# zju3dv/Diffuman4D

Measured on NVIDIA H100. Metric: unet_window_denoise_steps_per_sec, higher is better.
Workload: dtype bf16

## Files before the change

### diffuman4d_b200/_lib.py

```python
from __future__ import annotations

import ctypes as C
import os

_HERE = os.path.dirname(os.path.abspath(__file__))
LIB_PATH = os.path.join(_HERE, "libd4d.so")

EXPORTS = [
    "d4d_last_error", "d4d_version", "d4d_create", "d4d_destroy", "d4d_load_weight", "d4d_finalize_weights",
    "d4d_num_weights", "d4d_weight_key", "d4d_unet_forward", "d4d_profile_forward", "d4d_workspace_bytes", "d4d_forward_launches",
    "d4d_denoise_window", "d4d_denoise_window_dpm", "d4d_assemble_input", "d4d_cfg_ddim_step", "d4d_cfg_dpm_step",
    "d4d_op_gemm", "d4d_op_gemm_kv_scatter", "d4d_op_conv3x3",
    "d4d_op_attention", "d4d_op_groupnorm", "d4d_op_conv3x3_groupnorm", "d4d_op_conv_resample", "d4d_op_layernorm", "d4d_op_pose_conv0", "d4d_op_pose_conv", "d4d_debug_tap", "d4d_exchange_alloc",
    "d4d_exchange_open", "d4d_unet_forward_sharded", "d4d_denoise_window_sharded", "d4d_denoise_window_dpm_sharded",
    "d4d_window_exchange", "d4d_op_window_scatter", "d4d_denoise_window_unipc", "d4d_cfg_unipc_step",
    "d4d_op_conv_tiled", "d4d_conv_tile_choice", "d4d_op_gemm_tiled", "d4d_gemm_tile_choice",
    "d4d_denoise_window_pndm", "d4d_cfg_pndm_step", "d4d_denoise_window_deis", "d4d_cfg_deis_step",
    "d4d_denoise_window_dpm_single", "d4d_cfg_dpm_single_step",
    "d4d_denoise_window_cfg_split", "d4d_denoise_window_dpm_cfg_split", "d4d_denoise_window_unipc_cfg_split",
    "d4d_denoise_window_pndm_cfg_split", "d4d_denoise_window_deis_cfg_split", "d4d_denoise_window_dpm_single_cfg_split",
    "d4d_denoise_window_cfg_grid", "d4d_denoise_window_dpm_cfg_grid", "d4d_denoise_window_unipc_cfg_grid",
    "d4d_denoise_window_pndm_cfg_grid", "d4d_denoise_window_deis_cfg_grid", "d4d_denoise_window_dpm_single_cfg_grid",
]


class D4DConfig(C.Structure):
    _fields_ = [
        ("in_channels", C.c_int32), ("out_channels", C.c_int32), ("block_out_channels", C.c_int32 * 4),
        ("layers_per_block", C.c_int32), ("num_heads", C.c_int32 * 4), ("has_attn2", C.c_int32 * 4),
        ("use_linear_projection", C.c_int32), ("norm_num_groups", C.c_int32), ("norm_eps", C.c_float),
        ("flip_sin_to_cos", C.c_int32), ("freq_shift", C.c_float), ("num_3d_attn_blocks", C.c_int32),
# ... 99 lines not shown
    l.d4d_assemble_input.argtypes = [vp, vp, vp, vp, vp, vp, vp, i32, i32, i32, i32, i32, vp, vp, vp]
    l.d4d_cfg_ddim_step.argtypes = [vp, vp, vp, vp, vp, C.POINTER(D4DSched), f32, i32, i32, i32, i32, vp, vp]
    l.d4d_cfg_dpm_step.argtypes = [vp, vp, vp, vp, vp, vp, vp, vp, C.POINTER(D4DDpmSched), f32, i32, i32, i32, i32, vp, vp]
    l.d4d_cfg_unipc_step.argtypes = [vp, vp, vp, vp, vp, vp, vp, vp, vp, vp, C.POINTER(D4DUniPCSched), f32, i32, i32, i32,
                                     i32, vp, vp]
    l.d4d_cfg_pndm_step.argtypes = [vp, vp, vp, vp, vp, vp, vp, vp, vp, vp, vp, vp, C.POINTER(D4DPndmSched), f32, i32,
                                    i32, i32, i32, vp, vp]
    l.d4d_cfg_deis_step.argtypes = [vp, vp, vp, vp, vp, vp, vp, vp, vp, C.POINTER(D4DDeisSched), f32, i32, i32, i32, i32,
                                    vp, vp]
    l.d4d_cfg_dpm_single_step.argtypes = [vp, vp, vp, vp, vp, vp, vp, vp, vp, vp, C.POINTER(D4DDpmSingleSched), f32, i32,
                                          i32, i32, i32, vp, vp]
    l.d4d_op_gemm.argtypes = [vp, i32, i32, vp, i32, i32, vp, i32, i32, f32p, vp, i32, i32, vp, i32, vp, i32, i32,
                              i32, f32, i32, vp, i32, vp]
    l.d4d_op_gemm_tiled.argtypes = [vp, i32, i32, vp, i32, i32, vp, i32, i32, f32p, vp, i32, i32, vp, i32, vp, i32, i32,
                                    i32, f32, i32, i32, vp, i32, vp]
    l.d4d_gemm_tile_choice.argtypes = [i32, i32, i32, i32, i32, i32, C.POINTER(C.c_int), C.POINTER(C.c_int)]
    l.d4d_op_gemm_kv_scatter.argtypes = [vp, i32, i32, vp, i32, i32, vp, i32, i32, i32, C.c_int64, C.c_int64, C.c_int64,
                                         i32, vp, i32, vp]
    l.d4d_op_conv3x3.argtypes = [vp, i32, i32, i32, i32, vp, i32, f32p, vp, i32, vp, i32, vp, i32, vp, vp]
    l.d4d_op_conv_tiled.argtypes = [vp, i32, i32, i32, i32, vp, i32, f32p, vp, i32, vp, i32, vp, i32, i32, i32, vp, vp]
    l.d4d_conv_tile_choice.argtypes = [i32, i32, i32, i32, i32, i32, i32, C.POINTER(C.c_int), C.POINTER(C.c_int)]
    l.d4d_op_attention.argtypes = [vp, vp, vp, i32, vp, i32, i32, i32, i32, i32, f32, i32, i32, vp]
    l.d4d_op_groupnorm.argtypes = [vp, i32, vp, i32, i32, i32, i32, f32, f32p, f32p, i32, vp, vp, vp]
    l.d4d_op_conv3x3_groupnorm.argtypes = [vp, i32, i32, i32, i32, vp, i32, f32p, vp, i32, f32, f32p, f32p, i32, vp, vp, vp,
                                           vp]
    l.d4d_op_conv_resample.argtypes = [vp, i32, i32, i32, i32, vp, i32, f32p, i32, i32, i32, vp, vp, vp]
    l.d4d_op_layernorm.argtypes = [vp, i32, i32, f32, f32p, f32p, vp, vp]
    l.d4d_op_pose_conv0.argtypes = [vp, i32, i32, i32, vp, f32p, vp, vp]
    l.d4d_op_pose_conv.argtypes = [vp, i32, i32, i32, i32, vp, f32p, i32, i32, i32, vp, vp]
    l.d4d_debug_tap.argtypes = [vp, vp, vp, vp, C.POINTER(C.c_int32), i32, i32, i32, i32, i32, i32, vp, C.c_char_p,
                                C.POINTER(C.c_int32), vp]
# ... 30 lines not shown
```

### diffuman4d_b200/csrc/d4d_api.cu

```cuda
#include <new>
#include <stdexcept>

#include "unet.h"

namespace d4d {
static thread_local std::string g_last_error;
void set_error(const std::string& msg) { g_last_error = msg; }
}

struct d4d_handle {
  d4d::Model* model;
};

using d4d::bf16;

#define D4D_API_BEGIN try {
#define D4D_API_END                                        \
  }                                                        \
  catch (const std::bad_alloc&) {                          \
    d4d::set_error("out of host memory");                  \
    return 2;                                              \
  }                                                        \
  catch (const std::exception& e) {                        \
    d4d::set_error(std::string("internal error: ") + e.what()); \
// ... 105 lines not shown
  d4d::StepArgs a;
  const int hw = height * width;
  a.noise = static_cast<const bf16*>(noise); a.latents = static_cast<const bf16*>(latents);
  a.mask = static_cast<const bf16*>(cond_mask);
  a.timestep_indices = reinterpret_cast<const long long*>(timestep_indices);
  a.F = F; a.chw = 4 * hw; a.hw = hw; a.cfg = cfg; a.guidance = guidance_scale;
  a.out = static_cast<bf16*>(latents_out);
  a.ts_out = reinterpret_cast<long long*>(timestep_indices_out);
  return a;
}
}

extern "C" {

const char* d4d_last_error(void) { return d4d::g_last_error.c_str(); }
int d4d_version(void) { return 114; }

int d4d_create(const d4d_config* cfg, int device, d4d_handle** out) {
  D4D_API_BEGIN
  D4D_REQUIRE(cfg != nullptr && out != nullptr, "null argument");
  *out = nullptr;
  D4D_REQUIRE(cfg->layers_per_block >= 1 && cfg->layers_per_block <= 4, "layers_per_block");
  D4D_REQUIRE(cfg->out_channels >= 1 && cfg->out_channels <= 16, "out_channels must be in [1,16]");
  D4D_REQUIRE(cfg->in_channels >= 1 && cfg->in_channels <= 16, "in_channels must be in [1,16]");
  D4D_REQUIRE(cfg->norm_num_groups >= 1 && cfg->norm_num_groups <= 64, "norm_num_groups");
  for (int i = 0; i < 4; ++i) {
    const int c = cfg->block_out_channels[i], hds = cfg->num_heads[i];
    D4D_REQUIRE(c > 0 && c % 64 == 0, "block_out_channels must be positive multiples of 64");
    D4D_REQUIRE(c % cfg->norm_num_groups == 0, "channels must be divisible by norm_num_groups");
    D4D_REQUIRE(hds > 0 && c % hds == 0, "channels must be divisible by the number of heads");
    D4D_REQUIRE(c / hds <= 192 && (c / hds) % 8 == 0, "head_dim must be a multiple of 8 and <= 192");
// ... 247 lines not shown
  D4D_API_END
}

int d4d_op_gemm(const void* A, int lda, int K1, const void* A2, int lda2, int K2, const void* W, int M, int N,
                const float* bias, const void* rowvec, int ld_rowvec, int rows_per_image, const void* residual,
                int ld_res, void* out, int ldo, int geglu, int act, float out_scale, int block_n, int64_t* stats,
                int stats_rows, void* stream) {
  return d4d_op_gemm_tiled(A, lda, K1, A2, lda2, K2, W, M, N, bias, rowvec, ld_rowvec, rows_per_image, residual, ld_res, out,
                           ldo, geglu, act, out_scale, block_n, 0, stats, stats_rows, stream);
}

int d4d_op_gemm_tiled(const void* A, int lda, int K1, const void* A2, int lda2, int K2, const void* W, int M, int N,
                      const float* bias, const void* rowvec, int ld_rowvec, int rows_per_image, const void* residual,
                      int ld_res, void* out, int ldo, int geglu, int act, float out_scale, int block_n, int schedule,
                      int64_t* stats, int stats_rows, void* stream) {
  D4D_API_BEGIN
  d4d::GemmDesc d;
  d.A = static_cast<const bf16*>(A); d.lda = lda; d.K1 = K1;
  d.A2 = static_cast<const bf16*>(A2); d.lda2 = lda2; d.K2 = K2;
  d.Wt = static_cast<const bf16*>(W); d.M = M; d.N = N; d.bias = bias;
  d.rowvec = static_cast<const bf16*>(rowvec); d.ld_rowvec = ld_rowvec; d.rows_per_image = rows_per_image;
  d.residual = static_cast<const bf16*>(residual); d.ld_res = ld_res;
  d.out = static_cast<bf16*>(out); d.ldo = ldo; d.geglu = geglu; d.act = act; d.out_scale = out_scale; d.block_n = block_n;
  d.schedule = schedule;
  d.stats = reinterpret_cast<long long*>(stats); d.stats_rows = stats_rows;
  D4D_REQUIRE(M > 0, "empty GEMM");
  d4d::GemmLaunch L;
  if (int rc = d4d::gemm_prepare(d, &L)) return rc;
  return d4d::gemm_run(L, static_cast<cudaStream_t>(stream));
  D4D_API_END
}

int d4d_gemm_tile_choice(int M, int N, int K1, int K2, int geglu, int sms, int* block_n, int* schedule) {
  D4D_API_BEGIN
  D4D_REQUIRE(M > 0 && N > 0 && K1 > 0 && K2 >= 0 && sms > 0 && block_n && schedule, "gemm_tile_choice arguments");
  d4d::GemmDesc d;
  D4D_REQUIRE(K2 == 0 || K1 % 64 == 0, "two-source GEMM needs K1 % 64 == 0");
  d.M = M; d.N = N; d.K1 = K1 + K2; d.geglu = geglu;
  int block_m = 0;
  return d4d::gemm_choose_tile(d, sms, &block_m, block_n, schedule);
  D4D_API_END
}

int d4d_op_gemm_kv_scatter(const void* A, int lda, int K, const void* W, int M, int N, void* out, int ldo, int kv_col0,
                           int kv_ld, int64_t rows_local, int64_t rows_global, int64_t row_offset, int world,
                           void* const* kv_dst, int block_n, void* stream) {
  D4D_API_BEGIN
  D4D_REQUIRE(M > 0, "empty GEMM");
  D4D_REQUIRE(world >= 1 && world <= 8, "K/V scatter: world must be in [1, 8]");
  D4D_REQUIRE(kv_dst != nullptr, "K/V scatter: null destination buffer");
  d4d::GemmDesc d;
  d.A = static_cast<const bf16*>(A); d.lda = lda; d.K1 = K; d.Wt = static_cast<const bf16*>(W); d.M = M; d.N = N;
  d.out = static_cast<bf16*>(out); d.ldo = ldo; d.block_n = block_n;
  d.kv_world = world; d.kv_col0 = kv_col0; d.kv_ld = kv_ld;
  d.kv_rows_local = rows_local; d.kv_rows_global = rows_global; d.kv_row_offset = row_offset;
// ... 348 lines not shown
```

### diffuman4d_b200/csrc/gemm_wgmma.cu

```cuda
#include "kernels.h"
#include "wgmma.cuh"

namespace d4d {

namespace {

constexpr int BLOCK_M = 128;
constexpr int BLOCK_K = 64;
constexpr int A_BYTES = BLOCK_M * BLOCK_K * 2;
constexpr int BAR_BYTES = 1024;
constexpr int NUM_THREADS = 384;
constexpr int MAX_SMEM = 227 * 1024;

constexpr int SLAB_COLS = 32;
constexpr int SLAB_BYTES = 64 * SLAB_COLS * 2;

template <int BN, int MI, bool kStaged, bool kPingPong>
struct GemmCfg {
  static constexpr int TILE_A_BYTES = kPingPong ? A_BYTES : MI * A_BYTES;
  static constexpr int STAGE_BYTES = TILE_A_BYTES + BN * BLOCK_K * 2;
  static constexpr int STAGING_BYTES = kStaged ? 2 * 64 * MI * BN * 2 : 0;
  static constexpr int STAGES_FIT = (MAX_SMEM - 1024 - BAR_BYTES - STAGING_BYTES) / STAGE_BYTES;
  static constexpr int STAGES = STAGES_FIT > 8 ? 8 : STAGES_FIT;
  static constexpr int SMEM = 1024 + BAR_BYTES + STAGES * STAGE_BYTES + STAGING_BYTES;
};

struct TileCoord {
  int m0;
  int n_img0, y0, x0;
  int pa, pb;
};

template <bool kConv>
__device__ __forceinline__ void tile_coords(const GemmKernelArgs& a, int m_tile, TileCoord& t) {
  if (!kConv) {
    t.m0 = m_tile * BLOCK_M;
    t.n_img0 = t.y0 = t.x0 = 0;
    t.pa = t.pb = 0;
  } else {
    const int ph = a.n_phases > 1 ? m_tile / a.tiles_per_phase : 0;
    m_tile -= ph * a.tiles_per_phase;
    t.pa = ph >> 1;
    t.pb = ph & 1;
    int tx = m_tile % a.tiles_x;
    int r = m_tile / a.tiles_x;
    int ty = r % a.tiles_y;
    int tn = r / a.tiles_y;
    t.m0 = 0;
    t.x0 = tx * a.BW;
    t.y0 = ty * a.BH;
    t.n_img0 = tn * a.BN;
  }
}

template <bool kConv>
__device__ __forceinline__ void row_of(const GemmKernelArgs& a, const TileCoord& tc, int rr, long long& row, int& img,
// ... 13 lines not shown
    img = n;
  }
}

enum : int { E_BIAS = 1, E_ROWVEC = 2, E_ACT = 4, E_RES = 8, E_STATS = 16, E_KV = 32, E_ALL = 63, E_STAGED_ALL = E_ALL & ~E_KV };
__host__ __device__ constexpr bool gemm_staged(bool conv, int epi) { return !conv && !(epi & E_KV); }

constexpr int ORDER_BAR = 3;

template <int BN, int MI, bool kGeglu, bool kConv, int kEpi, bool kPingPong>
__global__ void __launch_bounds__(NUM_THREADS, 1)
gemm_wgmma_kernel(const __grid_constant__ CUtensorMap tmap_a, const __grid_constant__ CUtensorMap tmap_a2,
                  const __grid_constant__ CUtensorMap tmap_b, const __grid_constant__ CUtensorMap tmap_c,
                  const __grid_constant__ CUtensorMap tmap_r, const GemmKernelArgs a) {
  constexpr bool kStaged = gemm_staged(kConv, kEpi);
  static_assert(MI == 1 || (kConv && MI == 2) || kPingPong, "256-row tiles: conv mode only (a plain tile is 128 rows)");
  static_assert(!kPingPong || (kStaged && MI == 2), "ping-pong: staged plain GEMMs, one warpgroup per 128-row tile");
  using Cfg = GemmCfg<BN, MI, kStaged, kPingPong>;
  constexpr int STAGES = Cfg::STAGES;
  extern __shared__ uint8_t smem_raw[];
  uint8_t* smem = reinterpret_cast<uint8_t*>((reinterpret_cast<uintptr_t>(smem_raw) + 1023) & ~uintptr_t(1023));
  uint64_t* full = reinterpret_cast<uint64_t*>(smem);
  uint64_t* empty = full + STAGES;
  uint64_t* res_full = empty + STAGES;
  uint8_t* ring = smem + BAR_BYTES;

  const int warp = __shfl_sync(0xffffffffu, threadIdx.x >> 5, 0);
  const int lane = threadIdx.x & 31;
  const int total_tiles = a.m_tiles * a.n_tiles;

  if (threadIdx.x == 0) {
// ... 45 lines not shown
      }
    }
    return;
  }

  setmaxnreg_inc<232>();
  const int wg = (warp >> 2) - 1;
  const int wq = warp & 3;
  const bool wg_leader = (threadIdx.x & 127) == 0;
  const int wg_row0 = kPingPong ? 0 : wg * 64 * MI;
  const int r_base = wg_row0 + wq * 16 + (lane >> 2);
  const int c_base = 2 * (lane & 3);
  const uint32_t ring_u32 = smem_u32(ring);
  constexpr int STG_BLOCK = 64 * BN * 2;
  const bool staged = kStaged && a.staged;
  uint8_t* stg = ring + STAGES * Cfg::STAGE_BYTES + wg * MI * STG_BLOCK;
  const uint32_t stg_u32 = smem_u32(stg) + (r_base - wg_row0) * 64 + c_base * 2;
  const int stg_xor = (lane >> 3) & 3;
  const bool has_res = (kEpi & E_RES) && !kGeglu && a.residual != nullptr;
  const int out_cols = kGeglu ? a.N / 2 : a.N;
  uint32_t res_phase = 0;

  int stage = 0;
  uint32_t phase = 0;
  const auto skip_stages = [&](int n) {
    stage += n;
    while (stage >= STAGES) { stage -= STAGES; phase ^= 1; }
  };
  if (kPingPong && wg == 1) {
    skip_stages(a.k_blocks);
    named_barrier_arrive(ORDER_BAR, 256);
  }
  const int tile_step = kPingPong ? 2 * gridDim.x : gridDim.x;
  float acc[MI][BN / 2];
  for (int tile = blockIdx.x + (kPingPong ? wg * gridDim.x : 0); tile < total_tiles; tile += tile_step) {
    const int m_tile = tile / a.n_tiles;
    const int n_tile = tile % a.n_tiles;
    TileCoord tc;
    tile_coords<kConv>(a, m_tile, tc);
    const int n0 = n_tile * a.block_n;
    const int ocol0 = kGeglu ? n0 / 2 : n0;
    const int ocols = min(kGeglu ? a.block_n / 2 : a.block_n, out_cols - ocol0);
    const int n_slabs = (ocols + SLAB_COLS - 1) / SLAB_COLS;
    const int orow0 = tc.m0 + wg_row0;
    const int live_blocks = staged ? max(0, min(MI, (a.M - orow0 + 63) / 64)) : 0;

    if (kPingPong) named_barrier_sync(ORDER_BAR + wg, 256);
    int prev_stage = -1;
    for (int kb = 0; kb < a.k_blocks; ++kb) {
      mbar_wait_nocall(&full[stage], phase);
      const uint32_t sa = ring_u32 + stage * Cfg::STAGE_BYTES + wg_row0 * 128;
      const uint32_t sb = ring_u32 + stage * Cfg::STAGE_BYTES + Cfg::TILE_A_BYTES;
      const uint64_t adesc = make_wgmma_desc(sa, 16, 1024);
      const uint64_t bdesc = make_wgmma_desc(sb, 16, 1024);
      wgmma_fence();
#pragma unroll
      for (int k = 0; k < BLOCK_K / 16; ++k) {
        const int scale_d = (kb | k) != 0 ? 1 : 0;
#pragma unroll
        for (int mi = 0; mi < MI; ++mi) {
          const uint64_t ad = adesc + 512 * mi + 2 * k, bd = bdesc + 2 * k;
          if constexpr (BN == 64) wgmma_ss_n64(acc[mi], ad, bd, scale_d);
          else if constexpr (BN == 128) wgmma_ss_n128(acc[mi], ad, bd, scale_d);
          else if constexpr (BN == 160) wgmma_ss_n160(acc[mi], ad, bd, scale_d);
          else if constexpr (BN == 192) wgmma_ss_n192(acc[mi], ad, bd, scale_d);
          else wgmma_ss_n256(acc[mi], ad, bd, scale_d);
        }
      }
      wgmma_commit();
      if (kb == 0 && staged && wg_leader) {
        bulk_wait_group_read<0>();
        if (has_res && live_blocks > 0) {
          mbar_expect_tx(&res_full[wg], live_blocks * n_slabs * SLAB_BYTES);
          for (int mi = 0; mi < live_blocks; ++mi)
            for (int s = 0; s < n_slabs; ++s)
              tma_load_2d(stg + mi * STG_BLOCK + s * SLAB_BYTES, &tmap_r, &res_full[wg], ocol0 + s * SLAB_COLS, orow0 + 64 * mi);
        }
      }
      wgmma_wait<1>();
      if (prev_stage >= 0 && wg_leader) mbar_arrive(&empty[prev_stage]);
      prev_stage = stage;
      if (++stage == STAGES) { stage = 0; phase ^= 1; }
    }
    if (kPingPong) {
      if (tile + gridDim.x < total_tiles) named_barrier_arrive(ORDER_BAR + (wg ^ 1), 256);
      skip_stages(a.k_blocks);
    }
    wgmma_wait<0>();
#pragma unroll
    for (int mi = 0; mi < MI; ++mi) wgmma_fence_regs(acc[mi]);
    if (wg_leader) mbar_arrive(&empty[prev_stage]);

    if (staged) {
      named_barrier_sync(1 + wg, 128);
      if (has_res && live_blocks > 0) {
        mbar_wait_nocall(&res_full[wg], res_phase);
        res_phase ^= 1;
      }
    }
#pragma unroll
    for (int mi = 0; mi < MI; ++mi) {
      auto stg_addr = [&](int j, int h) {
        return stg_u32 + mi * STG_BLOCK + h * 8 * 64 + (j >> 2) * SLAB_BYTES + (((j & 3) ^ stg_xor) << 4);
      };
      float (&accm)[BN / 2] = acc[mi];
      long long rows[2];
      int imgs[2];
      bool valid[2];
      row_of<kConv>(a, tc, r_base + 64 * mi, rows[0], imgs[0], valid[0]);
      row_of<kConv>(a, tc, r_base + 64 * mi + 8, rows[1], imgs[1], valid[1]);
      if constexpr (kGeglu) {
        const bool has_bias = (kEpi & E_BIAS) && a.bias != nullptr;
#pragma unroll
        for (int p = 0; p < BN / 16; ++p) {
          if (16 * p >= a.block_n || n0 + 16 * p >= a.N) break;
          float2 ba = make_float2(0.f, 0.f), bg = make_float2(0.f, 0.f);
          if (has_bias) {
            ba = __ldg(reinterpret_cast<const float2*>(a.bias + n0 + 16 * p + c_base));
// ... 67 lines not shown
              s0 += __shfl_xor_sync(0xffffffffu, s0, m);
              s1 += __shfl_xor_sync(0xffffffffu, s1, m);
              q0 += __shfl_xor_sync(0xffffffffu, q0, m);
              q1 += __shfl_xor_sync(0xffffffffu, q1, m);
            }
            if (stats_on && lane < 4) {
              unsigned long long* st = reinterpret_cast<unsigned long long*>(a.stats) + (static_cast<size_t>(stats_img) * a.N + col) * 2;
              atomicAdd(st + 0, static_cast<unsigned long long>(__float2ll_rn(s0 * kGnSumScale)));
              atomicAdd(st + 1, static_cast<unsigned long long>(__float2ll_rn(q0 * kGnSqScale)));
              atomicAdd(st + 2, static_cast<unsigned long long>(__float2ll_rn(s1 * kGnSumScale)));
              atomicAdd(st + 3, static_cast<unsigned long long>(__float2ll_rn(q1 * kGnSqScale)));
            }
          }
        }
      }
    }
    if (staged) {
      fence_proxy_async_smem();
      named_barrier_sync(1 + wg, 128);
      if (wg_leader && live_blocks > 0) {
        for (int mi = 0; mi < live_blocks; ++mi)
          for (int s = 0; s < n_slabs; ++s)
            tma_store_2d(&tmap_c, stg + mi * STG_BLOCK + s * SLAB_BYTES, ocol0 + s * SLAB_COLS, orow0 + 64 * mi);
        bulk_commit_group();
      }
    }
  }
  if (staged && wg_leader) bulk_wait_group<0>();
}

}

namespace {

void conv_out_grid(const GemmDesc& d, int* oh, int* ow, int* phases) {
  *oh = d.conv_kind == 1 ? d.H / 2 : d.H;
  *ow = d.conv_kind == 1 ? d.W / 2 : d.W;
  *phases = d.conv_kind == 3 ? 4 : 1;
}
// ... 8 lines not shown
  return t;
}

}

constexpr int kOperandWeight = 128;
constexpr int kMinKBlocks256 = 16;
constexpr int kEpilogueWeight = 3072;

namespace {
bool pingpong_width(int bn, bool geglu) { return bn == 128 || (bn == 64 && !geglu); }
}

int gemm_choose_tile(const GemmDesc& d, int sms, int* block_m, int* block_n, int* schedule) {
  D4D_REQUIRE(d.block_m == 0 || d.block_m == 128 || d.block_m == 256, "block_m must be 0 (automatic), 128 or 256");
  D4D_REQUIRE(d.block_m != 256 || d.conv, "256-row tiles: convolutions only (a plain GEMM stages a 128-row tile for its TMA store)");
  D4D_REQUIRE(d.block_m != 256 || d.block_n <= 0 || d.block_n == 128 || d.block_n == 160,
              "256-row tiles run at block_n 128 or 160 (the accumulators of wider tiles do not fit the register file)");
  D4D_REQUIRE(d.schedule == 0 || d.schedule == kSchedCooperative || d.schedule == kSchedPingPong,
              "schedule must be 0 (automatic), 1 (cooperative) or 2 (ping-pong)");
  const bool pp_ok = !d.conv && d.kv_world == 0;
  D4D_REQUIRE(d.schedule != kSchedPingPong || pp_ok, "ping-pong: plain GEMMs without the K/V scatter only");
  D4D_REQUIRE(d.schedule != kSchedPingPong || d.block_n <= 0 || pingpong_width(d.block_n, d.geglu),
              "ping-pong runs at block_n 64 or 128 (GEGLU: 128; wider accumulators do not fit the register file)");
  int oh = 0, ow = 0, phases = 1;
  if (d.conv) conv_out_grid(d, &oh, &ow, &phases);
  D4D_REQUIRE(!d.conv || (d.n_img > 0 && oh > 0 && ow > 0), "empty conv");
  const auto best_tile = [&](bool pingpong, int* bm, int* bn) {
    long long best_cost = -1;
    for (int r : {128, 256}) {
      if (d.block_m > 0 ? r != d.block_m : (r == 256 && !d.conv)) continue;
      if (pingpong && r != 128) continue;
      const int k_blocks = d.conv ? (d.conv_kind >= 2 ? 4 : 9) * ((d.Cin + BLOCK_K - 1) / BLOCK_K) : 0;
      const long long m_tiles = d.conv ? conv_tile(r, d.n_img, oh, ow).tiles * phases : (static_cast<long long>(d.M) + r - 1) / r;
      for (int c : {64, 128, 160, 192, 256}) {
        if (d.block_n > 0) c = d.block_n;
        else if ((d.geglu && c % 64 != 0) || (pingpong && !pingpong_width(c, d.geglu))) continue;
        const long long n_tiles = (d.N + c - 1) / c, tiles = m_tiles * n_tiles;
        const bool fits = r == 128 || ((c == 128 || c == 160) && (d.block_m == 256 || (tiles >= sms && k_blocks >= kMinKBlocks256)));
        if (fits) {
          const long long waves = (tiles + sms - 1) / sms;
          const long long cost = waves * (static_cast<long long>(r) * c + kOperandWeight * (r + c)) + (n_tiles * c - d.N) * (r / 2);
          if (best_cost < 0 || cost <= best_cost) { best_cost = cost; *bm = r; *bn = c; }
        }
        if (d.block_n > 0) break;
      }
    }
    return best_cost >= 0;
  };
  const auto plain_time = [&](bool pingpong, int bn) {
    const long long k_blocks = (d.K1 + BLOCK_K - 1) / BLOCK_K + (d.A2 ? (d.K2 + BLOCK_K - 1) / BLOCK_K : 0);
    const long long tiles = ((static_cast<long long>(d.M) + BLOCK_M - 1) / BLOCK_M) * ((d.N + bn - 1) / bn);
    const long long per_sm = (tiles + sms - 1) / sms;
    const long long main = k_blocks * (static_cast<long long>(BLOCK_M) * bn + kOperandWeight * (BLOCK_M + bn));
    const long long epi = static_cast<long long>(kEpilogueWeight) * bn;
    return pingpong ? per_sm * std::max(main, epi) + std::min(main, epi) : per_sm * (main + epi);
  };
  int sched = d.schedule;
  if (sched == 0) {
    int pbm = 0, pbn = 0, cbm = 0, cbn = 0;
    const bool pp_fits = pp_ok && (d.block_n <= 0 || pingpong_width(d.block_n, d.geglu)) && best_tile(true, &pbm, &pbn) &&
                         d.N % pbn == 0;
    D4D_REQUIRE(best_tile(false, &cbm, &cbn), "no tile for this block_m / block_n");
    sched = pp_fits && plain_time(true, pbn) < plain_time(false, cbn) ? kSchedPingPong : kSchedCooperative;
  }
  D4D_REQUIRE(best_tile(sched == kSchedPingPong, block_m, block_n), "no tile for this block_m / block_n");
  if (schedule) *schedule = sched;
  return 0;
}

bool gemm_stats_fusable(const GemmDesc& d, int sms, const char** why) {
  const auto refuse = [&](const char* msg) {
    if (why) *why = msg;
    return false;
  };
  if (d.geglu || d.kv_world != 0) return refuse("GroupNorm statistics: plain / conv epilogue only");
  if (!d.conv) {
// ... 53 lines not shown
  a.kv_world = d.kv_world;
  a.kv_col0 = d.kv_col0;
  a.kv_ld = d.kv_ld;
  a.kv_rows_local = d.kv_rows_local > 0 ? d.kv_rows_local : 1;
  a.kv_rows_global = d.kv_rows_global;
  a.kv_row_offset = d.kv_row_offset;
  for (int i = 0; i < 8; ++i) a.kv_dst[i] = d.kv_dst[i];
  D4D_REQUIRE(d.ldo % 8 == 0 && (d.residual == nullptr || d.ld_res % 8 == 0) &&
              (d.rowvec == nullptr || d.ld_rowvec % 8 == 0), "leading dimensions must be multiples of 8");

  if (!d.conv) {
    D4D_REQUIRE(d.K1 > 0 && d.K1 % 8 == 0 && d.K2 % 8 == 0, "K must be a multiple of 8");
    D4D_REQUIRE(d.A2 == nullptr || d.K1 % BLOCK_K == 0, "two-source GEMM needs K1 % 64 == 0");
    a.mode = 0;
    a.M = d.M;
    a.m_tiles = (d.M + BLOCK_M - 1) / BLOCK_M;
    a.kb_split = (d.K1 + BLOCK_K - 1) / BLOCK_K;
    const int kb2 = d.A2 ? (d.K2 + BLOCK_K - 1) / BLOCK_K : 0;
    a.k_blocks = a.kb_split + kb2;
    const int K = d.K1 + (d.A2 ? d.K2 : 0);
    if (int rc = make_tmap_2d(&L->tmap_a, d.A, d.M, d.K1, d.lda, BLOCK_K, BLOCK_M, 128)) return rc;
    if (d.A2) {
      if (int rc = make_tmap_2d(&L->tmap_a2, d.A2, d.M, d.K2, d.lda2, BLOCK_K, BLOCK_M, 128)) return rc;
    } else {
      L->tmap_a2 = L->tmap_a;
    }
    if (int rc = make_tmap_2d(&L->tmap_b, d.Wt, d.N, K, K, BLOCK_K, bn, 128)) return rc;
    const auto aligned16 = [](const void* p) { return (reinterpret_cast<uintptr_t>(p) & 15) == 0; };
    a.staged = d.kv_world == 0 && (d.geglu ? bn % (2 * SLAB_COLS) : bn % SLAB_COLS) == 0 && aligned16(d.out) &&
               (d.residual == nullptr || aligned16(d.residual));
    D4D_REQUIRE(d.schedule != kSchedPingPong || a.staged, "ping-pong needs the staged epilogue (16-byte aligned out / residual)");
    a.pingpong = a.staged && sched == kSchedPingPong;
    L->tmap_c = L->tmap_r = L->tmap_a;
    if (a.staged) {
      if (int rc = make_tmap_2d(&L->tmap_c, d.out, d.M, d.geglu ? d.N / 2 : d.N, d.ldo, SLAB_COLS, 64, 64)) return rc;
      if (d.residual && !d.geglu)
        if (int rc = make_tmap_2d(&L->tmap_r, d.residual, d.M, d.N, d.ld_res, SLAB_COLS, 64, 64)) return rc;
    }
// ... 24 lines not shown
      else { a.H = d.H; a.W = d.W; }
      a.out_H = a.H; a.out_W = a.W;
    }
    a.M = d.n_img * a.H * a.W;
    a.cin_blocks = (d.Cin + BLOCK_K - 1) / BLOCK_K;
    a.k_blocks = a.n_taps * a.cin_blocks;
    a.kb_split = a.k_blocks;
    const ConvTile ct = conv_tile(bm, d.n_img, a.H, a.W);
    const int bw = ct.bw, bh = ct.bh, bnimg = ct.bn_img;
    D4D_REQUIRE(bw * bh * bnimg == bm && bnimg <= 256, "conv tile shape");
    a.BW = bw; a.BH = bh; a.BN = bnimg;
    a.tiles_x = (a.W + bw - 1) / bw;
    a.tiles_y = (a.H + bh - 1) / bh;
    a.tiles_per_phase = static_cast<int>(ct.tiles);
    a.m_tiles = a.tiles_per_phase * a.n_phases;
    a.M *= a.n_phases;
    if (int rc = make_tmap_nhwc(&L->tmap_a, d.A, d.n_img, d.H, d.W, d.Cin, BLOCK_K, bw, bh, bnimg, 128, a.in_stride)) return rc;
    L->tmap_a2 = L->tmap_c = L->tmap_r = L->tmap_a;
    const uint64_t kw = static_cast<uint64_t>(a.n_taps) * d.Cin;
    if (int rc = make_tmap_2d(&L->tmap_b, d.Wt, static_cast<uint64_t>(d.N) * a.n_phases, kw, kw, BLOCK_K, bn, 128)) return rc;
  }
  const int total = a.m_tiles * a.n_tiles;
  L->grid = total < sms ? total : sms;
  return 0;
}

namespace {

using GemmKernelFn = void (*)(const CUtensorMap, const CUtensorMap, const CUtensorMap, const CUtensorMap,
                              const CUtensorMap, const GemmKernelArgs);
// ... 3 lines not shown
  int epi;
  bool pingpong;
  GemmKernelFn fn;
  int smem;
};
#define D4D_GV_M(BN, MI, G, C, E) \
  {BN, 128 * MI, G, C, E, false, gemm_wgmma_kernel<BN, MI, G, C, E, false>, GemmCfg<BN, MI, gemm_staged(C, E), false>::SMEM}
#define D4D_GV(BN, G, C, E) D4D_GV_M(BN, 1, G, C, E)
#define D4D_GV_PP(BN, G, E) \
  {BN, 128, G, false, E, true, gemm_wgmma_kernel<BN, 2, G, false, E, true>, GemmCfg<BN, 2, true, true>::SMEM}
#define D4D_GV_PLAIN(BN, GV)                                                                                          \
                                         \
  GV(BN, false, 0), GV(BN, false, E_BIAS), GV(BN, false, E_BIAS | E_RES), GV(BN, false, E_BIAS | E_RES | E_STATS),     \
  GV(BN, false, GV##_ALL)
#define D4D_GV_COOP_ALL E_ALL
#define D4D_GV_PP_ALL E_STAGED_ALL
#define D4D_GV_COOP(BN, G, E) D4D_GV(BN, G, false, E)
#define D4D_GV_CONV(BN, MI)                                                                                           \
                                                            \
  D4D_GV_M(BN, MI, false, true, E_BIAS | E_ROWVEC | E_STATS), D4D_GV_M(BN, MI, false, true, E_BIAS | E_RES | E_STATS), \
  D4D_GV_M(BN, MI, false, true, E_BIAS | E_STATS), D4D_GV_M(BN, MI, false, true, E_ALL)
const GemmVariant kGemmVariants[] = {
    D4D_GV_PLAIN(128, D4D_GV_COOP), D4D_GV_CONV(128, 1), D4D_GV_CONV(128, 2), D4D_GV(128, true, false, E_BIAS),
    D4D_GV_PLAIN(160, D4D_GV_COOP), D4D_GV_CONV(160, 1), D4D_GV_CONV(160, 2),
    D4D_GV_PLAIN(192, D4D_GV_COOP),
    D4D_GV_PLAIN(256, D4D_GV_COOP), D4D_GV_CONV(256, 1), D4D_GV(256, true, false, E_BIAS),
    D4D_GV(64, false, false, E_ALL), D4D_GV(64, false, true, E_ALL), D4D_GV(64, true, false, E_BIAS),
    D4D_GV_PLAIN(128, D4D_GV_PP), D4D_GV_PP(128, true, E_BIAS), D4D_GV_PP(64, false, E_STAGED_ALL),
};
#undef D4D_GV_COOP
#undef D4D_GV_COOP_ALL
#undef D4D_GV_PP_ALL
#undef D4D_GV_CONV
#undef D4D_GV_PLAIN
#undef D4D_GV_PP
#undef D4D_GV
#undef D4D_GV_M
constexpr int kNumGemmVariants = sizeof(kGemmVariants) / sizeof(kGemmVariants[0]);

int gemm_variant_at(const GemmKernelArgs& a, int bn) {
  const bool conv = a.mode != 0, geglu = a.geglu != 0;
  int need = 0;
  if (a.bias) need |= E_BIAS;
  if (!geglu) {
    if (a.rowvec) need |= E_ROWVEC;
    if (a.act == 1 || a.out_scale != 1.0f) need |= E_ACT;
// ... 43 lines not shown
```

### diffuman4d_b200/csrc/kernels.h

```cpp
#pragma once
#include <cstdlib>
#include <mutex>
#include <utility>
#include <string.h>

#include "../../include/d4d.h"
#include "common.cuh"

namespace d4d {

constexpr float kGnSumScale = 268435456.f;
constexpr float kGnSqScale = 16777216.f;

struct GemmKernelArgs {
  int M, N, k_blocks, block_n, n_tiles, m_tiles;
  int block_m;
  int mode;
  int kb_split;
  int H, W, n_img, Cin, cin_blocks, BW, BH, BN, tiles_x, tiles_y;
  int n_taps, in_stride, out_sy, out_sx, out_oy, out_ox, out_H, out_W;
  int n_phases, tiles_per_phase;
  signed char tap_dy[9], tap_dx[9];
  const float* bias;
  const bf16* rowvec;
  int ld_rowvec, rows_per_image;
  const bf16* residual;
  int ld_res;
  bf16* out;
  int ldo;
  int staged;
  int pingpong;
  int geglu;
  int act;
  float out_scale;
  long long* stats;
  int stats_rows;
// ... 212 lines not shown
```

### include/d4d.h

```cpp
#ifndef D4D_H_
#define D4D_H_

#include <stddef.h>
#include <stdint.h>

#ifdef __cplusplus
extern "C" {
#endif

typedef struct d4d_handle d4d_handle;

typedef struct d4d_config {
  int32_t in_channels;
  int32_t out_channels;
  int32_t block_out_channels[4];
  int32_t layers_per_block;
  int32_t num_heads[4];
  int32_t has_attn2[4];
  int32_t use_linear_projection;
  int32_t norm_num_groups;
  float norm_eps;
  int32_t flip_sin_to_cos;
  float freq_shift;
  int32_t num_3d_attn_blocks;
// ... 147 lines not shown
                int stats_rows, void* stream);
int d4d_op_gemm_kv_scatter(const void* A, int lda, int K, const void* W, int M, int N, void* out, int ldo, int kv_col0,
                           int kv_ld, int64_t rows_local, int64_t rows_global, int64_t row_offset, int world,
                           void* const* kv_dst, int block_n, void* stream);
int d4d_op_conv3x3(const void* x_nhwc, int n_img, int H, int W, int Cin, const void* Wt, int Cout, const float* bias,
                   const void* rowvec, int ld_rowvec, const void* residual, int act, void* out, int block_n,
                   int64_t* stats, void* stream);
int d4d_op_conv_tiled(const void* x_nhwc, int n_img, int H, int W, int Cin, const void* Wt, int Cout, const float* bias,
                      const void* rowvec, int ld_rowvec, const void* residual, int act, void* out, int kind, int block_m,
                      int block_n, int64_t* stats, void* stream);
int d4d_conv_tile_choice(int n_img, int H, int W, int Cin, int Cout, int kind, int sms, int* block_m, int* block_n);
int d4d_op_gemm_tiled(const void* A, int lda, int K1, const void* A2, int lda2, int K2, const void* W, int M, int N,
                      const float* bias, const void* rowvec, int ld_rowvec, int rows_per_image, const void* residual,
                      int ld_res, void* out, int ldo, int geglu, int act, float out_scale, int block_n, int schedule,
                      int64_t* stats, int stats_rows, void* stream);
int d4d_gemm_tile_choice(int M, int N, int K1, int K2, int geglu, int sms, int* block_n, int* schedule);
int d4d_op_attention(const void* q, const void* k, const void* v, int ld_qkv, void* out, int ld_out, int batch,
                     int seq, int heads, int head_dim, float scale, int seq_kv, int ld_kv, void* stream);
int d4d_op_groupnorm(const void* x1, int C1, const void* x2, int C2, int n_img, int hw, int groups, float eps,
                     const float* gamma, const float* beta, int silu, void* out, int64_t* stats, void* stream);
int d4d_op_conv_resample(const void* x_nhwc, int n_img, int H, int W, int Cin, const void* Wt, int Cout, const float* bias,
                         int kind, int up_a, int up_b, void* out, int64_t* stats, void* stream);
int d4d_op_conv3x3_groupnorm(const void* x_nhwc, int n_img, int H, int W, int Cin, const void* Wt, int Cout,
                             const float* bias, const void* residual, int groups, float eps, const float* gamma,
                             const float* beta, int silu, void* conv_out, void* gn_out, int64_t* stats, void* stream);
int d4d_op_layernorm(const void* x, int rows, int C, float eps, const float* gamma, const float* beta, void* out,
                     void* stream);
int d4d_op_pose_conv0(const void* x_nchw, int n, int H, int W, const void* Wt, const float* bias, void* out_nhwc4,
                      void* stream);
int d4d_op_pose_conv(const void* x_nhwc, int n, int Cin, int H, int W, const void* Wt, const float* bias, int Cout,
                     int ksize, int stride, void* out, void* stream);
// ... 89 lines not shown
```

Measured before the change: 14.52.

## Enable 256-row tiles for plain GEMMs and group-ordered M tile scheduling

Allows plain (non-GEGLU, non-scatter) cooperative GEMMs to use 256-row tiles at block_n 128 by staging the epilogue one 64-row slab at a time, loading residuals and storing per slab so the staging buffer stays small. It also adds an m_order remap that interleaves M tiles across stats groups (images) when statistics are collected, changing tile traversal order. The auto tile chooser can now pick 256-row plain tiles when there are enough tiles and K blocks, trading more register pressure and serialized per-slab epilogue barriers for larger operand reuse.

```diff
diff --git a/diffuman4d_b200/_lib.py b/diffuman4d_b200/_lib.py
--- a/diffuman4d_b200/_lib.py
+++ b/diffuman4d_b200/_lib.py
@@ -15,6 +15,7 @@
     "d4d_exchange_open", "d4d_unet_forward_sharded", "d4d_denoise_window_sharded", "d4d_denoise_window_dpm_sharded",
     "d4d_window_exchange", "d4d_op_window_scatter", "d4d_denoise_window_unipc", "d4d_cfg_unipc_step",
     "d4d_op_conv_tiled", "d4d_conv_tile_choice", "d4d_op_gemm_tiled", "d4d_gemm_tile_choice",
+    "d4d_op_gemm_tiled_rows", "d4d_gemm_tile_choice_rows",
     "d4d_denoise_window_pndm", "d4d_cfg_pndm_step", "d4d_denoise_window_deis", "d4d_cfg_deis_step",
     "d4d_denoise_window_dpm_single", "d4d_cfg_dpm_single_step",
     "d4d_denoise_window_cfg_split", "d4d_denoise_window_dpm_cfg_split", "d4d_denoise_window_unipc_cfg_split",
@@ -144,7 +145,11 @@
                               i32, f32, i32, vp, i32, vp]
     l.d4d_op_gemm_tiled.argtypes = [vp, i32, i32, vp, i32, i32, vp, i32, i32, f32p, vp, i32, i32, vp, i32, vp, i32, i32,
                                     i32, f32, i32, i32, vp, i32, vp]
+    l.d4d_op_gemm_tiled_rows.argtypes = [vp, i32, i32, vp, i32, i32, vp, i32, i32, f32p, vp, i32, i32, vp, i32, vp, i32,
+                                         i32, i32, f32, i32, i32, i32, vp, i32, vp]
     l.d4d_gemm_tile_choice.argtypes = [i32, i32, i32, i32, i32, i32, C.POINTER(C.c_int), C.POINTER(C.c_int)]
+    l.d4d_gemm_tile_choice_rows.argtypes = [i32, i32, i32, i32, i32, i32, C.POINTER(C.c_int), C.POINTER(C.c_int),
+                                            C.POINTER(C.c_int)]
     l.d4d_op_gemm_kv_scatter.argtypes = [vp, i32, i32, vp, i32, i32, vp, i32, i32, i32, C.c_int64, C.c_int64, C.c_int64,
                                          i32, vp, i32, vp]
     l.d4d_op_conv3x3.argtypes = [vp, i32, i32, i32, i32, vp, i32, f32p, vp, i32, vp, i32, vp, i32, vp, vp]
diff --git a/diffuman4d_b200/csrc/d4d_api.cu b/diffuman4d_b200/csrc/d4d_api.cu
--- a/diffuman4d_b200/csrc/d4d_api.cu
+++ b/diffuman4d_b200/csrc/d4d_api.cu
@@ -143,7 +143,7 @@
 extern "C" {
 
 const char* d4d_last_error(void) { return d4d::g_last_error.c_str(); }
-int d4d_version(void) { return 114; }
+int d4d_version(void) { return 115; }
 
 int d4d_create(const d4d_config* cfg, int device, d4d_handle** out) {
   D4D_API_BEGIN
@@ -421,6 +421,14 @@
                       const float* bias, const void* rowvec, int ld_rowvec, int rows_per_image, const void* residual,
                       int ld_res, void* out, int ldo, int geglu, int act, float out_scale, int block_n, int schedule,
                       int64_t* stats, int stats_rows, void* stream) {
+  return d4d_op_gemm_tiled_rows(A, lda, K1, A2, lda2, K2, W, M, N, bias, rowvec, ld_rowvec, rows_per_image, residual, ld_res,
+                                out, ldo, geglu, act, out_scale, 0, block_n, schedule, stats, stats_rows, stream);
+}
+
+int d4d_op_gemm_tiled_rows(const void* A, int lda, int K1, const void* A2, int lda2, int K2, const void* W, int M, int N,
+                           const float* bias, const void* rowvec, int ld_rowvec, int rows_per_image, const void* residual,
+                           int ld_res, void* out, int ldo, int geglu, int act, float out_scale, int block_m, int block_n,
+                           int schedule, int64_t* stats, int stats_rows, void* stream) {
   D4D_API_BEGIN
   d4d::GemmDesc d;
   d.A = static_cast<const bf16*>(A); d.lda = lda; d.K1 = K1;
@@ -428,8 +436,8 @@
   d.Wt = static_cast<const bf16*>(W); d.M = M; d.N = N; d.bias = bias;
   d.rowvec = static_cast<const bf16*>(rowvec); d.ld_rowvec = ld_rowvec; d.rows_per_image = rows_per_image;
   d.residual = static_cast<const bf16*>(residual); d.ld_res = ld_res;
-  d.out = static_cast<bf16*>(out); d.ldo = ldo; d.geglu = geglu; d.act = act; d.out_scale = out_scale; d.block_n = block_n;
-  d.schedule = schedule;
+  d.out = static_cast<bf16*>(out); d.ldo = ldo; d.geglu = geglu; d.act = act; d.out_scale = out_scale;
+  d.block_m = block_m; d.block_n = block_n; d.schedule = schedule;
   d.stats = reinterpret_cast<long long*>(stats); d.stats_rows = stats_rows;
   D4D_REQUIRE(M > 0, "empty GEMM");
   d4d::GemmLaunch L;
@@ -439,13 +447,17 @@
 }
 
 int d4d_gemm_tile_choice(int M, int N, int K1, int K2, int geglu, int sms, int* block_n, int* schedule) {
-  D4D_API_BEGIN
-  D4D_REQUIRE(M > 0 && N > 0 && K1 > 0 && K2 >= 0 && sms > 0 && block_n && schedule, "gemm_tile_choice arguments");
+  int block_m = 0;
+  return d4d_gemm_tile_choice_rows(M, N, K1, K2, geglu, sms, &block_m, block_n, schedule);
+}
+
+int d4d_gemm_tile_choice_rows(int M, int N, int K1, int K2, int geglu, int sms, int* block_m, int* block_n, int* schedule) {
+  D4D_API_BEGIN
+  D4D_REQUIRE(M > 0 && N > 0 && K1 > 0 && K2 >= 0 && sms > 0 && block_m && block_n && schedule, "gemm_tile_choice arguments");
   d4d::GemmDesc d;
   D4D_REQUIRE(K2 == 0 || K1 % 64 == 0, "two-source GEMM needs K1 % 64 == 0");
   d.M = M; d.N = N; d.K1 = K1 + K2; d.geglu = geglu;
-  int block_m = 0;
-  return d4d::gemm_choose_tile(d, sms, &block_m, block_n, schedule);
+  return d4d::gemm_choose_tile(d, sms, block_m, block_n, schedule);
   D4D_API_END
 }
 
diff --git a/diffuman4d_b200/csrc/gemm_wgmma.cu b/diffuman4d_b200/csrc/gemm_wgmma.cu
--- a/diffuman4d_b200/csrc/gemm_wgmma.cu
+++ b/diffuman4d_b200/csrc/gemm_wgmma.cu
@@ -19,7 +19,8 @@
 struct GemmCfg {
   static constexpr int TILE_A_BYTES = kPingPong ? A_BYTES : MI * A_BYTES;
   static constexpr int STAGE_BYTES = TILE_A_BYTES + BN * BLOCK_K * 2;
-  static constexpr int STAGING_BYTES = kStaged ? 2 * 64 * MI * BN * 2 : 0;
+  static constexpr int SLAB_SETS = kPingPong ? MI : 1;
+  static constexpr int STAGING_BYTES = kStaged ? 2 * SLAB_SETS * 64 * BN * 2 : 0;
   static constexpr int STAGES_FIT = (MAX_SMEM - 1024 - BAR_BYTES - STAGING_BYTES) / STAGE_BYTES;
   static constexpr int STAGES = STAGES_FIT > 8 ? 8 : STAGES_FIT;
   static constexpr int SMEM = 1024 + BAR_BYTES + STAGES * STAGE_BYTES + STAGING_BYTES;
@@ -31,15 +32,19 @@
   int pa, pb;
 };
 
+__device__ __forceinline__ int m_order(const GemmKernelArgs& a, int m) {
+  return a.m_groups > 1 ? (m % a.m_groups) * a.m_group_tiles + m / a.m_groups : m;
+}
+
 template <bool kConv>
 __device__ __forceinline__ void tile_coords(const GemmKernelArgs& a, int m_tile, TileCoord& t) {
   if (!kConv) {
-    t.m0 = m_tile * BLOCK_M;
+    t.m0 = m_order(a, m_tile) * a.block_m;
     t.n_img0 = t.y0 = t.x0 = 0;
     t.pa = t.pb = 0;
   } else {
     const int ph = a.n_phases > 1 ? m_tile / a.tiles_per_phase : 0;
-    m_tile -= ph * a.tiles_per_phase;
+    m_tile = m_order(a, m_tile - ph * a.tiles_per_phase);
     t.pa = ph >> 1;
     t.pb = ph & 1;
     int tx = m_tile % a.tiles_x;
@@ -83,7 +88,7 @@
                   const __grid_constant__ CUtensorMap tmap_b, const __grid_constant__ CUtensorMap tmap_c,
                   const __grid_constant__ CUtensorMap tmap_r, const GemmKernelArgs a) {
   constexpr bool kStaged = gemm_staged(kConv, kEpi);
-  static_assert(MI == 1 || (kConv && MI == 2) || kPingPong, "256-row tiles: conv mode only (a plain tile is 128 rows)");
+  static_assert(MI == 1 || MI == 2, "a warpgroup owns one or two 64-row blocks");
   static_assert(!kPingPong || (kStaged && MI == 2), "ping-pong: staged plain GEMMs, one warpgroup per 128-row tile");
   using Cfg = GemmCfg<BN, MI, kStaged, kPingPong>;
   constexpr int STAGES = Cfg::STAGES;
@@ -159,12 +164,30 @@
   const uint32_t ring_u32 = smem_u32(ring);
   constexpr int STG_BLOCK = 64 * BN * 2;
   const bool staged = kStaged && a.staged;
-  uint8_t* stg = ring + STAGES * Cfg::STAGE_BYTES + wg * MI * STG_BLOCK;
+  constexpr int SLAB_SETS = Cfg::SLAB_SETS;
+  uint8_t* stg = ring + STAGES * Cfg::STAGE_BYTES + wg * SLAB_SETS * STG_BLOCK;
   const uint32_t stg_u32 = smem_u32(stg) + (r_base - wg_row0) * 64 + c_base * 2;
   const int stg_xor = (lane >> 3) & 3;
   const bool has_res = (kEpi & E_RES) && !kGeglu && a.residual != nullptr;
   const int out_cols = kGeglu ? a.N / 2 : a.N;
   uint32_t res_phase = 0;
+  struct StagedTile { int ocol0, n_slabs, orow0, live_blocks; };
+  const auto staged_tile = [&](int tile) {
+    StagedTile t;
+    const int n0 = (tile % a.n_tiles) * a.block_n;
+    t.ocol0 = kGeglu ? n0 / 2 : n0;
+    t.n_slabs = (min(kGeglu ? a.block_n / 2 : a.block_n, out_cols - t.ocol0) + SLAB_COLS - 1) / SLAB_COLS;
+    t.orow0 = m_order(a, tile / a.n_tiles) * a.block_m + wg_row0;
+    t.live_blocks = max(0, min(MI, (a.M - t.orow0 + 63) / 64));
+    return t;
+  };
+  const auto load_residual = [&](const StagedTile& t, int mi0, int mi1) {
+    mbar_expect_tx(&res_full[wg], (mi1 - mi0) * t.n_slabs * SLAB_BYTES);
+    for (int mi = mi0; mi < mi1; ++mi)
+      for (int s = 0; s < t.n_slabs; ++s)
+        tma_load_2d(stg + (mi % SLAB_SETS) * STG_BLOCK + s * SLAB_BYTES, &tmap_r, &res_full[wg], t.ocol0 + s * SLAB_COLS,
+                    t.orow0 + 64 * mi);
+  };
 
   int stage = 0;
   uint32_t phase = 0;
@@ -184,11 +207,6 @@
     TileCoord tc;
     tile_coords<kConv>(a, m_tile, tc);
     const int n0 = n_tile * a.block_n;
-    const int ocol0 = kGeglu ? n0 / 2 : n0;
-    const int ocols = min(kGeglu ? a.block_n / 2 : a.block_n, out_cols - ocol0);
-    const int n_slabs = (ocols + SLAB_COLS - 1) / SLAB_COLS;
-    const int orow0 = tc.m0 + wg_row0;
-    const int live_blocks = staged ? max(0, min(MI, (a.M - orow0 + 63) / 64)) : 0;
 
     if (kPingPong) named_barrier_sync(ORDER_BAR + wg, 256);
     int prev_stage = -1;
@@ -215,11 +233,9 @@
       wgmma_commit();
       if (kb == 0 && staged && wg_leader) {
         bulk_wait_group_read<0>();
-        if (has_res && live_blocks > 0) {
-          mbar_expect_tx(&res_full[wg], live_blocks * n_slabs * SLAB_BYTES);
-          for (int mi = 0; mi < live_blocks; ++mi)
-            for (int s = 0; s < n_slabs; ++s)
-              tma_load_2d(stg + mi * STG_BLOCK + s * SLAB_BYTES, &tmap_r, &res_full[wg], ocol0 + s * SLAB_COLS, orow0 + 64 * mi);
+        if (has_res) {
+          const StagedTile st = staged_tile(tile);
+          if (st.live_blocks > 0) load_residual(st, 0, SLAB_SETS > 1 ? st.live_blocks : 1);
         }
       }
       wgmma_wait<1>();
@@ -236,17 +252,25 @@
     for (int mi = 0; mi < MI; ++mi) wgmma_fence_regs(acc[mi]);
     if (wg_leader) mbar_arrive(&empty[prev_stage]);
 
-    if (staged) {
-      named_barrier_sync(1 + wg, 128);
-      if (has_res && live_blocks > 0) {
-        mbar_wait_nocall(&res_full[wg], res_phase);
-        res_phase ^= 1;
-      }
-    }
+    const StagedTile st = staged_tile(tile);
 #pragma unroll
     for (int mi = 0; mi < MI; ++mi) {
+      if (staged) {
+        if (mi >= st.live_blocks) break;
+        if (mi == 0 || SLAB_SETS == 1) {
+          if (mi > 0 && wg_leader) {
+            bulk_wait_group_read<0>();
+            if (has_res) load_residual(st, mi, mi + 1);
+          }
+          named_barrier_sync(1 + wg, 128);
+          if (has_res) {
+            mbar_wait_nocall(&res_full[wg], res_phase);
+            res_phase ^= 1;
+          }
+        }
+      }
       auto stg_addr = [&](int j, int h) {
-        return stg_u32 + mi * STG_BLOCK + h * 8 * 64 + (j >> 2) * SLAB_BYTES + (((j & 3) ^ stg_xor) << 4);
+        return stg_u32 + (mi % SLAB_SETS) * STG_BLOCK + h * 8 * 64 + (j >> 2) * SLAB_BYTES + (((j & 3) ^ stg_xor) << 4);
       };
       float (&accm)[BN / 2] = acc[mi];
       long long rows[2];
@@ -344,15 +368,14 @@
           }
         }
       }
-    }
-    if (staged) {
-      fence_proxy_async_smem();
-      named_barrier_sync(1 + wg, 128);
-      if (wg_leader && live_blocks > 0) {
-        for (int mi = 0; mi < live_blocks; ++mi)
-          for (int s = 0; s < n_slabs; ++s)
-            tma_store_2d(&tmap_c, stg + mi * STG_BLOCK + s * SLAB_BYTES, ocol0 + s * SLAB_COLS, orow0 + 64 * mi);
-        bulk_commit_group();
+      if (staged) {
+        fence_proxy_async_smem();
+        named_barrier_sync(1 + wg, 128);
+        if (wg_leader) {
+          for (int s = 0; s < st.n_slabs; ++s)
+            tma_store_2d(&tmap_c, stg + (mi % SLAB_SETS) * STG_BLOCK + s * SLAB_BYTES, st.ocol0 + s * SLAB_COLS, st.orow0 + 64 * mi);
+          bulk_commit_group();
+        }
       }
     }
   }
@@ -391,9 +414,12 @@
 
 int gemm_choose_tile(const GemmDesc& d, int sms, int* block_m, int* block_n, int* schedule) {
   D4D_REQUIRE(d.block_m == 0 || d.block_m == 128 || d.block_m == 256, "block_m must be 0 (automatic), 128 or 256");
-  D4D_REQUIRE(d.block_m != 256 || d.conv, "256-row tiles: convolutions only (a plain GEMM stages a 128-row tile for its TMA store)");
-  D4D_REQUIRE(d.block_m != 256 || d.block_n <= 0 || d.block_n == 128 || d.block_n == 160,
-              "256-row tiles run at block_n 128 or 160 (the accumulators of wider tiles do not fit the register file)");
+  const bool plain256_ok = d.conv || (!d.geglu && d.kv_world == 0);
+  D4D_REQUIRE(d.block_m != 256 || plain256_ok, "256-row tiles: convolutions and plain GEMMs without GEGLU or the K/V scatter");
+  D4D_REQUIRE(d.block_m != 256 || d.schedule != kSchedPingPong, "ping-pong runs 128-row tiles");
+  D4D_REQUIRE(d.block_m != 256 || d.block_n <= 0 || d.block_n == 128 || (d.conv && d.block_n == 160),
+              "256-row tiles run at block_n 128, convs at 160 as well (the accumulators of wider tiles do not fit the register "
+              "file; a plain GEMM's staged epilogue spills at 160)");
   D4D_REQUIRE(d.schedule == 0 || d.schedule == kSchedCooperative || d.schedule == kSchedPingPong,
               "schedule must be 0 (automatic), 1 (cooperative) or 2 (ping-pong)");
   const bool pp_ok = !d.conv && d.kv_world == 0;
@@ -414,7 +440,8 @@
         if (d.block_n > 0) c = d.block_n;
         else if ((d.geglu && c % 64 != 0) || (pingpong && !pingpong_width(c, d.geglu))) continue;
         const long long n_tiles = (d.N + c - 1) / c, tiles = m_tiles * n_tiles;
-        const bool fits = r == 128 || ((c == 128 || c == 160) && (d.block_m == 256 || (tiles >= sms && k_blocks >= kMinKBlocks256)));
+        const bool fits = r == 128 || ((c == 128 || (c == 160 && d.conv)) &&
+                                       (d.block_m == 256 || (tiles >= sms && k_blocks >= kMinKBlocks256)));
         if (fits) {
           const long long waves = (tiles + sms - 1) / sms;
           const long long cost = waves * (static_cast<long long>(r) * c + kOperandWeight * (r + c)) + (n_tiles * c - d.N) * (r / 2);
@@ -436,8 +463,8 @@
   int sched = d.schedule;
   if (sched == 0) {
     int pbm = 0, pbn = 0, cbm = 0, cbn = 0;
-    const bool pp_fits = pp_ok && (d.block_n <= 0 || pingpong_width(d.block_n, d.geglu)) && best_tile(true, &pbm, &pbn) &&
-                         d.N % pbn == 0;
+    const bool pp_fits = pp_ok && d.block_m != 256 && (d.block_n <= 0 || pingpong_width(d.block_n, d.geglu)) &&
+                         best_tile(true, &pbm, &pbn) && d.N % pbn == 0;
     D4D_REQUIRE(best_tile(false, &cbm, &cbn), "no tile for this block_m / block_n");
     sched = pp_fits && plain_time(true, pbn) < plain_time(false, cbn) ? kSchedPingPong : kSchedCooperative;
   }
@@ -521,14 +548,19 @@
     D4D_REQUIRE(d.A2 == nullptr || d.K1 % BLOCK_K == 0, "two-source GEMM needs K1 % 64 == 0");
     a.mode = 0;
     a.M = d.M;
-    a.m_tiles = (d.M + BLOCK_M - 1) / BLOCK_M;
+    a.m_tiles = (d.M + bm - 1) / bm;
+    a.m_groups = 1;
+    if (d.stats && d.stats_rows % bm == 0) {
+      a.m_groups = d.M / d.stats_rows;
+      a.m_group_tiles = d.stats_rows / bm;
+    }
     a.kb_split = (d.K1 + BLOCK_K - 1) / BLOCK_K;
     const int kb2 = d.A2 ? (d.K2 + BLOCK_K - 1) / BLOCK_K : 0;
     a.k_blocks = a.kb_split + kb2;
     const int K = d.K1 + (d.A2 ? d.K2 : 0);
-    if (int rc = make_tmap_2d(&L->tmap_a, d.A, d.M, d.K1, d.lda, BLOCK_K, BLOCK_M, 128)) return rc;
+    if (int rc = make_tmap_2d(&L->tmap_a, d.A, d.M, d.K1, d.lda, BLOCK_K, bm, 128)) return rc;
     if (d.A2) {
-      if (int rc = make_tmap_2d(&L->tmap_a2, d.A2, d.M, d.K2, d.lda2, BLOCK_K, BLOCK_M, 128)) return rc;
+      if (int rc = make_tmap_2d(&L->tmap_a2, d.A2, d.M, d.K2, d.lda2, BLOCK_K, bm, 128)) return rc;
     } else {
       L->tmap_a2 = L->tmap_a;
     }
@@ -583,6 +615,11 @@
     a.tiles_y = (a.H + bh - 1) / bh;
     a.tiles_per_phase = static_cast<int>(ct.tiles);
     a.m_tiles = a.tiles_per_phase * a.n_phases;
+    a.m_groups = 1;
+    if (d.stats) {
+      a.m_groups = (d.n_img + bnimg - 1) / bnimg;
+      a.m_group_tiles = a.tiles_x * a.tiles_y;
+    }
     a.M *= a.n_phases;
     if (int rc = make_tmap_nhwc(&L->tmap_a, d.A, d.n_img, d.H, d.W, d.Cin, BLOCK_K, bw, bh, bnimg, 128, a.in_stride)) return rc;
     L->tmap_a2 = L->tmap_c = L->tmap_r = L->tmap_a;
@@ -616,14 +653,17 @@
   GV(BN, false, 0), GV(BN, false, E_BIAS), GV(BN, false, E_BIAS | E_RES), GV(BN, false, E_BIAS | E_RES | E_STATS),     \
   GV(BN, false, GV##_ALL)
 #define D4D_GV_COOP_ALL E_ALL
+#define D4D_GV_COOP256_ALL E_STAGED_ALL
 #define D4D_GV_PP_ALL E_STAGED_ALL
 #define D4D_GV_COOP(BN, G, E) D4D_GV(BN, G, false, E)
+#define D4D_GV_COOP256(BN, G, E) D4D_GV_M(BN, 2, G, false, E)
 #define D4D_GV_CONV(BN, MI)                                                                                           \
                                                             \
   D4D_GV_M(BN, MI, false, true, E_BIAS | E_ROWVEC | E_STATS), D4D_GV_M(BN, MI, false, true, E_BIAS | E_RES | E_STATS), \
   D4D_GV_M(BN, MI, false, true, E_BIAS | E_STATS), D4D_GV_M(BN, MI, false, true, E_ALL)
 const GemmVariant kGemmVariants[] = {
     D4D_GV_PLAIN(128, D4D_GV_COOP), D4D_GV_CONV(128, 1), D4D_GV_CONV(128, 2), D4D_GV(128, true, false, E_BIAS),
+    D4D_GV_PLAIN(128, D4D_GV_COOP256),
     D4D_GV_PLAIN(160, D4D_GV_COOP), D4D_GV_CONV(160, 1), D4D_GV_CONV(160, 2),
     D4D_GV_PLAIN(192, D4D_GV_COOP),
     D4D_GV_PLAIN(256, D4D_GV_COOP), D4D_GV_CONV(256, 1), D4D_GV(256, true, false, E_BIAS),
@@ -632,6 +672,8 @@
 };
 #undef D4D_GV_COOP
 #undef D4D_GV_COOP_ALL
+#undef D4D_GV_COOP256
+#undef D4D_GV_COOP256_ALL
 #undef D4D_GV_PP_ALL
 #undef D4D_GV_CONV
 #undef D4D_GV_PLAIN
diff --git a/diffuman4d_b200/csrc/kernels.h b/diffuman4d_b200/csrc/kernels.h
--- a/diffuman4d_b200/csrc/kernels.h
+++ b/diffuman4d_b200/csrc/kernels.h
@@ -20,6 +20,7 @@
   int H, W, n_img, Cin, cin_blocks, BW, BH, BN, tiles_x, tiles_y;
   int n_taps, in_stride, out_sy, out_sx, out_oy, out_ox, out_H, out_W;
   int n_phases, tiles_per_phase;
+  int m_groups, m_group_tiles;
   signed char tap_dy[9], tap_dx[9];
   const float* bias;
   const bf16* rowvec;
diff --git a/include/d4d.h b/include/d4d.h
--- a/include/d4d.h
+++ b/include/d4d.h
@@ -185,7 +185,12 @@
                       const float* bias, const void* rowvec, int ld_rowvec, int rows_per_image, const void* residual,
                       int ld_res, void* out, int ldo, int geglu, int act, float out_scale, int block_n, int schedule,
                       int64_t* stats, int stats_rows, void* stream);
+int d4d_op_gemm_tiled_rows(const void* A, int lda, int K1, const void* A2, int lda2, int K2, const void* W, int M, int N,
+                           const float* bias, const void* rowvec, int ld_rowvec, int rows_per_image, const void* residual,
+                           int ld_res, void* out, int ldo, int geglu, int act, float out_scale, int block_m, int block_n,
+                           int schedule, int64_t* stats, int stats_rows, void* stream);
 int d4d_gemm_tile_choice(int M, int N, int K1, int K2, int geglu, int sms, int* block_n, int* schedule);
+int d4d_gemm_tile_choice_rows(int M, int N, int K1, int K2, int geglu, int sms, int* block_m, int* block_n, int* schedule);
 int d4d_op_attention(const void* q, const void* k, const void* v, int ld_qkv, void* out, int ld_out, int batch,
                      int seq, int heads, int head_dim, float scale, int seq_kv, int ld_kv, void* stream);
 int d4d_op_groupnorm(const void* x1, int C1, const void* x2, int C2, int n_img, int hw, int groups, float eps,
```

After: 14.69, median of 6. +1.2%, better.
